# raadyn/aztotmd

Hardware: AMD Instinct MI355X
Metric: ns_per_day (higher is better)
Workload: dtype f64; 1 GPU; 1 000 188 Ar, LJ rc 8.5 A, FCC 63^3 a=5.735 jitter 0.15, dt 1 fs, NVE, init_vel zero (BASELINE config '1 000 000 Ar LJ', SURVEY C4); n_atoms=1000188, n_cells=68921, decomposition=single GPU, transport=single GPU, rccl_ranks=0, pair_variant=0, sort_interval=105, sort_violations=0, pair_lists=1, cells_without_list=0, kernel_timing=off

## Files before the change

### aztotmd_amd/api.py

```python
import ctypes as C
import enum
import os
import subprocess

import numpy as np

_HERE = os.path.dirname(os.path.abspath(__file__))
_LIB = None

STAT_FIELDS = ("step", "time", "engTot", "engKin", "engVdW", "engCoul", "engElecField", "engTemp", "engPot", "temperature",
               "posMom", "negMom", "posCross", "negCross", "pressure", "pairs_dropped", "n_cells", "nose_chit", "nose_conint",
               "engBond", "engAngle", "engCoulRec", "engCoulConst", "sort_interval", "sort_violations", "pair_lists", "cells_without_list", "rebuilds", "skin")


class AztotError(RuntimeError):
    def __init__(self, code, msg):
        super().__init__("aztot error %d: %s" % (code, msg))
        self.code = code


class _Species(C.Structure):
    _fields_ = [("name", C.c_char * 8), ("mass_amu", C.c_double), ("charge", C.c_double), ("frozen", C.c_int32),
                ("radA", C.c_double), ("radB", C.c_double), ("mxEng", C.c_double)]

# ... 85 lines not shown
EXPORTS = ("aztot_device_count", "aztot_device_synchronize", "aztot_init_md", "aztot_model_create", "aztot_model_set_bonded", "aztot_model_query", "aztot_model_species_name", "aztot_model_nucleus_name", "aztot_free_md", "aztot_default_options",
           "aztot_init_device", "aztot_free_device", "aztot_step", "aztot_sync", "aztot_forces", "aztot_get_stats", "aztot_species_crossings", "aztot_md_to_host",
           "aztot_set_state", "aztot_get_clock", "aztot_set_clock", "aztot_cell_table", "aztot_kernel_times", "aztot_reset_kernel_times", "aztot_set_profile", "aztot_comm_id_bytes", "aztot_comm_make_id", "aztot_comm_selftest", "aztot_comm_ranks",
           "aztot_init_device_slab", "aztot_rdf_setup", "aztot_rdf_sample", "aztot_rdf_reset", "aztot_rdf_shape", "aztot_rdf_counts", "aztot_rdf_values",
           "aztot_cn_setup", "aztot_cn_sample", "aztot_cn_shape", "aztot_cn_per_atom", "aztot_cn_table",
           "aztot_tcf_setup", "aztot_tcf_sample", "aztot_tcf_reset", "aztot_tcf_shape", "aztot_tcf_sums", "aztot_tcf_values",
           "aztot_stress_setup", "aztot_stress_sample", "aztot_stress_get", "aztot_stress_per_atom",
           "aztot_adf_setup", "aztot_adf_sample", "aztot_adf_reset", "aztot_adf_shape", "aztot_adf_edges", "aztot_adf_counts", "aztot_adf_values",
           "aztot_adf_neighbours",
           "aztot_sk_setup", "aztot_sk_sample", "aztot_sk_reset", "aztot_sk_shape", "aztot_sk_vectors", "aztot_sk_amplitudes", "aztot_sk_sums", "aztot_sk_values",
           "aztot_boo_setup", "aztot_boo_sample", "aztot_boo_reset", "aztot_boo_shape", "aztot_boo_per_atom", "aztot_boo_qlm", "aztot_boo_counts", "aztot_boo_values",
           "aztot_last_error", "aztot_version")

RDF_KINDS = {"species": 0, "nuclei": 1}
CN_KINDS = {"species": 0, "nuclei": 1}


class DebugBit(enum.IntFlag):
    DBG_BUILD_PHASE_MASK = 3
    DBG_ALWAYS_CLEANUP = 4
    DBG_FOLD_DRIFT = 8
    DBG_NO_FOLD_DRIFT = 16
    DBG_WIDE_ENTRIES = 32
    DBG_KICK_EVERY_STEP = 128
    DBG_LARGE_KICK_PATH = 256
    DBG_GENERIC_PAIR = 512
    DBG_KEEP_VDW_CUT_TEST = 1024
    DBG_STAGE_ONLY = 2048
    DBG_SLAB_GRAPH = 4096
    DBG_FIXED_INTERVAL = 8192
    DBG_OVERLAP_HALO = 16384
    DBG_NO_LISTS = 32768
    DBG_SHORT_LISTS = 65536
    DBG_NO_FUSE_NEXT = 131072
    DBG_FUSE_NEXT = 262144
    DBG_CHECK_EVERY_ATOM = 524288
    DBG_LIST_STATS = 2097152
    DBG_KICK_POST_SPLIT = 4194304
    DBG_GRAPH_ALWAYS = 8388608
    DBG_PLAIN_ONE_ATOM = 16777216
    DBG_NO_BOUNDARY_RADI = 33554432
    DBG_ONE_WAVE_PER_CELL = 67108864
    DBG_ENERGIES_EVERY_STEP = 134217728
    DBG_SETTLE_EVERY_CALL = 268435456
    DBG_NO_FOLD_KICK = 536870912
    DBG_FOLD_KICK = 1073741824
# ... 662 lines not shown
```

### aztotmd_amd/csrc/device_md.h

```cpp
#pragma once
#include <cstdint>

namespace aztot {

constexpr int kSpecCap = 16;

struct AtomArrays
{
    double *x, *y, *z;
    double *vx, *vy, *vz;
    double *fx, *fy, *fz;
    double *U, *rad;
    int32_t *type;
    int32_t *id;
};

struct RefPos { double *x, *y, *z; };

struct SpecTable
{
    double mass[kSpecCap], charge[kSpecCap], rMhdt[kSpecCap];
    double radA[kSpecCap], radB[kSpecCap], mxEng[kSpecCap];
    int32_t charged[kSpecCap], frozen[kSpecCap];
};
// ... 41 lines not shown
    const EwaldG* groups;
    double* T;
    int32_t nK, nW, nG, kx, ky, kz, nBlocksA;
    double* partial;
    double* S;
    double scale, scale2;
};

struct SplitArgs
{
    int n = 1;
    double *fx = nullptr, *fy = nullptr, *fz = nullptr;
    int32_t* arrived = nullptr;
    int capacity = 0;
};

enum DebugBit : unsigned
{
    DBG_BUILD_PHASE_MASK = 3,
    DBG_ALWAYS_CLEANUP = 4,
    DBG_FOLD_DRIFT = 8,
    DBG_NO_FOLD_DRIFT = 16,
    DBG_WIDE_ENTRIES = 32,
    DBG_KICK_EVERY_STEP = 128,
    DBG_LARGE_KICK_PATH = 256,
    DBG_GENERIC_PAIR = 512,
    DBG_KEEP_VDW_CUT_TEST = 1024,
    DBG_STAGE_ONLY = 2048,
    DBG_SLAB_GRAPH = 4096,
    DBG_FIXED_INTERVAL = 8192,
    DBG_OVERLAP_HALO = 16384,
    DBG_NO_LISTS = 32768,
    DBG_SHORT_LISTS = 65536,
    DBG_NO_FUSE_NEXT = 131072,
    DBG_FUSE_NEXT = 262144,
    DBG_CHECK_EVERY_ATOM = 524288,
    DBG_LIST_STATS = 2097152,
    DBG_KICK_POST_SPLIT = 4194304,
    DBG_GRAPH_ALWAYS = 8388608,
    DBG_PLAIN_ONE_ATOM = 16777216,
    DBG_NO_BOUNDARY_RADI = 33554432,
    DBG_ONE_WAVE_PER_CELL = 67108864,
    DBG_ENERGIES_EVERY_STEP = 134217728,
    DBG_SETTLE_EVERY_CALL = 268435456,
    DBG_NO_FOLD_KICK = 536870912,
    DBG_FOLD_KICK = 1073741824
// ... 99 lines not shown
```

### aztotmd_amd/csrc/engine.hip

```cpp
#include "engine.h"

#include <algorithm>
#include <cmath>
#include <array>
#include <cstring>
#include <cstddef>
#include <cstdio>
#include <cstdlib>
#include <stdexcept>
#include <tuple>

#include "exchange.h"
#include "bonded.hip.h"
#include "ewald.hip.h"
#include "kernels.hip.h"
#include "pair_tile.hip.h"
#include "pair_list.hip.h"
#include "rdf.hip.h"
#include "cn.hip.h"
#include "adf.hip.h"
#include "sk.hip.h"
#include "tcf.hip.h"
#include "slab.hip.h"

// ... 466 lines not shown
    waves = forcedWaves_ ? forcedWaves_ : waves_wanted(density * vol, 0);
    int cand = (int)(density * vol * 1.5) + 64;
    int iters = (int)(partners * 1.25 / list_slices(list_atoms_per_wave(std::min(kWave * waves, (int)(1.6 * perCell) + 6), waves))) + 4;
    cand = std::max(kListMinCand * waves, (cand + 63) & ~63);
    iters = std::max(2 * kListMinIter, (iters + 7) & ~7);
    if (const char* e = std::getenv("AZTOT_CAND_CAP")) cand = std::atoi(e);
    if (const char* e = std::getenv("AZTOT_ITER_CAP")) iters = std::atoi(e);
    try { allocate(cand, iters); }
    catch (const std::exception&)
    {
        (void)hipGetLastError();
        release();
    }
}

void ListStore::allocate(int candCapNew, int iterCapNew)
{
    release();
    const StepParams& P = *P_;
    candCapNew = std::max(kListMinCand * waves, std::min((candCapNew + 63) & ~63, kListCandMax));
    iterCapNew = std::max(kListMinIter, std::min((iterCapNew + 7) & ~7, kListIterMax));
    PairLists probe;
    probe.candCap = probe.candLds = probe.stageLds = candCapNew; probe.iterCap = probe.iterLds = iterCapNew; probe.recBytes = pair_list_rec_bytes(P); probe.waves = waves;
    while (candCapNew > kListMinCand && (pair_list_lds_bytes(P, probe) > ldsMax_ || build_lists_lds_bytes(probe) > ldsMax_))
    {
        candCapNew -= 64;
        probe.candCap = probe.candLds = probe.stageLds = candCapNew;
    }
    while (iterCapNew > 2 * kListMinIter && build_lists_lds_bytes(probe) > ldsMax_) { iterCapNew -= 8; probe.iterCap = probe.iterLds = iterCapNew; }
    const size_t nc = (size_t)P.nCellLocal;
    cand = mem_.alloc<uint32_t>(nc * candCapNew, true, stream_);
    meta = mem_.alloc<int32_t>(4 * nc, false, stream_);
    pairs = mem_.alloc<uint16_t>(nc * (size_t)waves * (size_t)iterCapNew * kWave, true, stream_);
    report = mem_.alloc<int32_t>(LR_COUNT, true, stream_); rel = mem_.alloc<float4>((size_t)capacity_ + kWave, true, stream_);
    candCap = candCapNew; iterCap = iterCapNew;
    candLds = stageLds = candCapNew; iterLds = iterCapNew;
    entryBytes = entryNext = 2;
    {
        std::vector<int32_t> mx(4 * nc, 0);
        const int ncy = P.nc[1], ncz = P.nc[2];
        for (size_t c = 0; c < nc; c++)
        {
            const int cz = (int)(c % ncz), cy = (int)((c / ncz) % ncy), lx = (int)(c / ((size_t)ncy * ncz));
            mx[4 * c] = -1; mx[4 * c + 1] = lx | (cy << 10) | (cz << 20);
        }
        HIP_CHECK(hipMemcpyAsync(meta, mx.data(), sizeof(int32_t) * 4 * nc, hipMemcpyHostToDevice, stream_));
        HIP_CHECK(hipStreamSynchronize(stream_));
    }
    on = true;
    if (std::getenv("AZTOT_VERBOSE"))
        std::fprintf(stderr, "aztot: pair lists for %zu cells: %d candidates, %d iterations per cell (%.1f MB), LDS %zu B (list kernel) / %zu B (builder)\n", nc, candCap, iterCap,
                     (double)(nc * ((size_t)candCap * 4 + (size_t)iterCap * 128)) / 1e6, pair_list_lds_bytes(P, pair_lists()), build_lists_lds_bytes(pair_lists()));
}

void ListStore::regrow(int candCapNew, int iterCapNew)
{
    try { allocate(candCapNew, iterCapNew); }
    catch (const std::exception& e)
    {
        (void)hipGetLastError();
        release();
        if (std::getenv("AZTOT_VERBOSE")) std::fprintf(stderr, "aztot: rank %d: no room for larger pair lists (%s): the run goes on without lists\n", rank_, e.what());
    }
}

void ListStore::release() noexcept
{
    if (stream_) (void)hipStreamSynchronize(stream_);
    mem_.release();
    cand = nullptr; meta = nullptr; pairs = nullptr; report = nullptr; rel = nullptr;
    on = false;
}

PairLists ListStore::pair_lists() const
{
    PairLists pl;
    if (on)
    {
        pl.cand = cand; pl.meta = meta; pl.pairs = pairs; pl.noList = report;
        pl.candCap = candCap; pl.iterCap = iterCap; pl.candLds = candLds; pl.stageLds = stageLds; pl.iterLds = iterLds; pl.recBytes = pair_list_rec_bytes(*P_); pl.waves = waves;
        pl.entryBytes = entryBytes; pl.entryScale = entryBytes == 1 ? 1 : pair_list_entry_scale(*P_);
        pl.rel = rel;
    }
    return pl;
}

int ListStore::tile_records_for(int maxT) const
{
    constexpr size_t kLdsBlock = 1280;
    PairLists L = pair_lists();
    const bool roomy = P_->nranks == 1 && capacity_ <= 2 * kFuseKickMaxAtoms;
    int need = std::max(4 * kWave, std::min(candCap, roomy ? maxT + maxT / 16 + 4 : maxT + maxT / 100 + 1));
    if (maxT <= 255 && P_->nranks == 1 && waves == 1) need = 4 * kWave;
    if (need <= 4 * kWave) return need;
    L.candLds = need;
    const size_t blocks = (pair_list_lds_bytes(*P_, L) + kLdsBlock - 1) / kLdsBlock;
    int best = need;
    for (int c = need + 1; c <= candCap; c++)
    {
        L.candLds = c;
        if ((pair_list_lds_bytes(*P_, L) + kLdsBlock - 1) / kLdsBlock > blocks) break;
        best = c;
    }
    return best;
}

int ListStore::stage_records_for(int maxStaged) const
{
    return std::max(4 * kWave, std::min(candCap, (maxStaged + maxStaged / 16 + 4 + 127) & ~127));
}

void ListStore::lds_for(const int32_t* rep, int& candLdsNew, int& stageLdsNew, int& iterLdsNew) const
{
    candLdsNew = tile_records_for(rep[LR_MAX_TILE]);
    stageLdsNew = stage_records_for(rep[LR_MAX_STAGED]);
    iterLdsNew = std::max(2 * kListMinIter, std::min(iterCap, (rep[LR_MAX_ITERS] + rep[LR_MAX_ITERS] / 8 + 2 + 7) & ~7));
    if (entryNext == 1 && ((iterLdsNew + 15) & ~15) <= iterCap) iterLdsNew = (iterLdsNew + 15) & ~15;
}

bool ListStore::narrow_fits(int maxTile, int candLdsNew, int wavesNew) const
{
    return P_->nranks == 1 && !(P_->debugMask & DBG_WIDE_ENTRIES) && !wideForGood_ && wavesNew == 1 && list_preload(candLdsNew) == 4 && maxTile <= 255;
}

bool ListStore::tighten(const int32_t* rep, bool* formatChanged)
{
    if (formatChanged) *formatChanged = false;
    if (rep[LR_TILE_FULL] != 0 || rep[LR_LIST_FULL] != 0 || rep[LR_KEPT_FULL] != 0 || rep[LR_MAX_STAGED] <= 0) return false;
    int c, s, i;
    lds_for(rep, c, s, i);
    bool changed = false;
    if (entryNext == 2 && narrow_fits(rep[LR_MAX_TILE], std::min(candLds, c), waves))
    {
        entryNext = 1;
        lds_for(rep, c, s, i);
        changed = true;
        if (formatChanged) *formatChanged = true;
    }
    if (c >= candLds && s >= stageLds && i >= iterLds) return changed;
    candLds = std::min(candLds, c); stageLds = std::min(stageLds, s); iterLds = std::min(iterLds, i);
    return true;
}

ListStore::Verdict ListStore::adapt(const int32_t* rep, unsigned debug)
{
    Verdict v;
    const bool frozen = debug & DBG_SHORT_LISTS;
    if (debug & DBG_LIST_STATS)
    {
        std::fprintf(stderr, "aztot: per cell: %.2f list iterations, %.1f candidates staged, %.1f kept, %.2f atoms; %.1f %% of the cells walk more than 16 iterations (%d-byte entries)\n",
                     (double)rep[LR_SUM_ITERS] / rep[LR_RECORDED], (double)rep[LR_SUM_STAGED] / rep[LR_RECORDED], (double)rep[LR_SUM_CANDS] / rep[LR_RECORDED],
                     (double)rep[LR_SUM_ATOMS] / rep[LR_RECORDED], 100.0 * (double)rep[LR_OVER_16] / rep[LR_RECORDED], entryBytes);
        HIP_CHECK(hipMemset(&report[LR_SUM_ITERS], 0, sizeof(int32_t) * 4));
        HIP_CHECK(hipMemset(&report[LR_OVER_16], 0, sizeof(int32_t)));
    }
    HIP_CHECK(hipMemsetAsync(&report[LR_UNLISTED], 0, sizeof(int32_t) * 2, stream_));
    HIP_CHECK(hipMemsetAsync(&report[LR_TILE_FULL], 0, sizeof(int32_t) * 3, stream_));
    const int tileFull = rep[LR_TILE_FULL], keptFull = rep[LR_KEPT_FULL], listFull = rep[LR_LIST_FULL], recorded = rep[LR_RECORDED], unlisted = rep[LR_UNLISTED];
    if (std::getenv("AZTOT_VERBOSE"))
        std::fprintf(stderr, "aztot: lists recorded since the last look: %d cells, %d of them without a list (%d: staging full, %d: tile full, %d: list full); most staged %d of %d (LDS %d), largest tile %d (LDS %d), longest list %d of %d (LDS %d)\n",
                     recorded, unlisted, tileFull, keptFull, listFull, rep[LR_MAX_STAGED], candCap, stageLds, rep[LR_MAX_TILE], candLds, rep[LR_MAX_ITERS], iterCap, iterLds);
    int candLdsNew, stageLdsNew, iterLdsNew;
    lds_for(rep, candLdsNew, stageLdsNew, iterLdsNew);
    if (tileFull > 0) stageLdsNew = std::min(candCap, std::max(stageLdsNew, stageLds + 128));
    if (keptFull > 0) candLdsNew = std::min(candCap, std::max(candLdsNew, candLds + 32));
    if (listFull > 0) iterLdsNew = std::min(iterCap, std::max(iterLdsNew, iterLds + 8));
    if (frozen) { candLdsNew = candLds; stageLdsNew = stageLds; iterLdsNew = iterLds; }
    const int wWant = std::max(waves, waves_wanted((double)rep[LR_MAX_TILE], rep[LR_MAX_ITERS]));
    const int wavesNew = (wWant > waves && !forcedWaves_ && !frozen) ? wWant : waves;
    if (entryNext == 1 && (rep[LR_MAX_TILE] > 255 || keptFull > 0 || !narrow_fits(rep[LR_MAX_TILE], candLdsNew, wavesNew)))
    {
        entryNext = 2; wideForGood_ = true;
        v.rebuild = v.launchChanged = true;
    }
    else if (entryNext == 2 && !frozen && tileFull + keptFull + listFull == 0 && narrow_fits(rep[LR_MAX_TILE], candLdsNew, wavesNew))
    {
        entryNext = 1;
        v.launchChanged = true;
        lds_for(rep, candLdsNew, stageLdsNew, iterLdsNew);
    }
    if (wWant > waves && !forcedWaves_ && !frozen)
    {
        const int itersNew = std::max(2 * kListMinIter, ((int)(rep[LR_MAX_ITERS] * (double)waves / wWant * 1.3) + 8 + 7) & ~7);
        const int candNew = std::max(candCap, kListMinCand * wWant);
        waves = wWant;
        regrow(candNew, itersNew);
        v.rebuild = v.launchChanged = true;
        return v;
    }
    const bool capFull = (tileFull > 0 && stageLds == candCap) || (keptFull > 0 && candLds == candCap) || (listFull > 0 && iterLds == iterCap);
    if (capFull && !frozen && (double)(tileFull + keptFull + listFull) > ((P_->nranks == 1 && growths < 3) ? 0.0 : 0.0005 * (double)recorded))
    {
        const int candNew = tileFull + keptFull > 0 ? std::min(kListCandMax, (candCap * 3 / 2 + 63) & ~63) : candCap;
        const int itersNew = listFull > 0 ? std::min(kListIterMax, (iterCap * 2 + 7) & ~7) : iterCap;
        v.launchChanged = true;
        if (growths < 3 && (candNew > candCap || itersNew > iterCap)) { growths++; regrow(candNew, itersNew); v.rebuild = true; }
    }
    else if (candLdsNew != candLds || stageLdsNew != stageLds || iterLdsNew != iterLds)
    {
        candLds = candLdsNew; stageLds = stageLdsNew; iterLds = iterLdsNew;
        v.launchChanged = true;
    }
    if (on && (double)unlisted > 0.02 * (double)recorded && !frozen && tileFull + keptFull + listFull < unlisted / 2)
    {
        on = false;
        v.launchChanged = true;
    }
    return v;
}

void Engine::upload_bonded()
{
    const Model& m = model_;
    const size_t nb = m.bondA.size(), na = m.angC.size();
    hasBonded_ = (nb + na) > 0;
    if (!hasBonded_) return;
    const int N = m.nAt;
    auto up = [&](const void* src, size_t bytes) {
        void* p = dev_alloc<char>(bytes);
        if (bytes) HIP_CHECK(hipMemcpy(p, src, bytes, hipMemcpyHostToDevice));
        return p;
    };
    std::vector<int32_t> bs(N + 1, 0), as(N + 1, 0);
    for (size_t k = 0; k < nb; k++) { bs[m.bondA[k] + 1]++; bs[m.bondB[k] + 1]++; }
    for (size_t k = 0; k < na; k++) { as[m.angC[k] + 1]++; as[m.angL1[k] + 1]++; as[m.angL2[k] + 1]++; }
    for (int i = 0; i < N; i++) { bs[i + 1] += bs[i]; as[i + 1] += as[i]; }
// ... 1118 lines not shown
```

### aztotmd_amd/csrc/list_store.h

```cpp
#pragma once
#include "device_resources.h"
#include "model.h"

namespace aztot {

struct StepParams; struct PairLists;

struct ListStore
{
    struct Verdict
    {
        bool rebuild = false;
        bool launchChanged = false;
    };

    bool on = false;
    uint32_t* cand = nullptr;
    int32_t* meta = nullptr;
    uint16_t* pairs = nullptr;
    int32_t* report = nullptr;
    float4* rel = nullptr;
    int candCap = 0, iterCap = 0;
    int candLds = 0, iterLds = 0;
    int stageLds = 0;
    int waves = 1;
    int growths = 0;
    int entryBytes = 2, entryNext = 2;

    void create(const StepParams& P, const Model& m, const aztot_options& opt, int capacity, double listRadius, hipStream_t stream, int rank);
    void regrow(int candCap, int iterCap);
    void release() noexcept;
    PairLists pair_lists() const;
    void lds_for(const int32_t* rep, int& candLds, int& stageLds, int& iterLds) const;
    bool tighten(const int32_t* rep, bool* formatChanged = nullptr);
    bool narrow_fits(int maxTile, int candLdsNew, int wavesNew) const;
    void begin_recording() { entryBytes = entryNext; }
    Verdict adapt(const int32_t* rep, unsigned debug);

private:
    void allocate(int candCap, int iterCap);
    int tile_records_for(int maxT) const;
    int stage_records_for(int maxStaged) const;
    int waves_wanted(double tileRecords, int iters) const;
    DeviceArena mem_;
    const StepParams* P_ = nullptr;
    hipStream_t stream_ = nullptr;
    int capacity_ = 0, rank_ = 0;
    int forcedWaves_ = 0;
    bool wideForGood_ = false;
    size_t ldsMax_ = 0;
};

}
```

### aztotmd_amd/csrc/pair_list.hip.h

```cpp
#pragma once
#include <type_traits>
#include "pair_tile.hip.h"

namespace aztot {

constexpr int kListPreload = 5;
constexpr int kListMinCand = 64 * kListPreload;
__host__ __device__ inline int list_preload(int candLds) { return candLds <= 4 * kWave ? 4 : kListPreload; }
constexpr int kListMinIter = 16;
constexpr int kListMaxSlices = 32;

constexpr int kListMaxWaves = 4;
__host__ __device__ inline int list_atoms_per_wave(int nAtoms, int W) { return (nAtoms + W - 1) >> (W >> 1); }
__host__ __device__ inline int list_slices(int nAtomsOfWave) { const int n = kWave / (nAtomsOfWave > 0 ? nAtomsOfWave : 1); return n > kListMaxSlices ? kListMaxSlices : (n < 1 ? 1 : n); }

inline bool pair_list_tab_mode(const StepParams& P) { return P.potSet == POTSET_ONE_FAMILY && !P.single_lj; }
inline size_t pair_list_lds_bytes(const StepParams& P, const PairLists& L)
{
    const bool tab = pair_list_tab_mode(P);
    const bool generic = !P.single_lj && P.potSet == POTSET_GENERIC;
    const bool radii = !P.single_lj && !tab;
    size_t b = (size_t)(L.candLds + 1) * 24;
    if (tab) b += sizeof(double) * kLjSpecMax * kLjSpecMax * kPairTabStride + (((size_t)L.candLds + 1 + 15) & ~(size_t)15);
    if (radii) b += sizeof(double) * (size_t)(L.candLds + 1);
// ... 349 lines not shown
            partials[(size_t)PS_EVDW * maxBlocks + pb] = eV;
            partials[(size_t)PS_ECOUL * maxBlocks + pb] = eC;
        }
        if (dropped != 0.0) partials[(size_t)PS_DROPPED * maxBlocks + pb] += dropped;
    }
    if (ENG && P.fuseKick == KICK_SECOND)
    {
        eK = wave_sum(eK);
        if (lane == 0) partials[(size_t)PS_EKIN * maxBlocks + pb] = 0.5 * eK;
    }
    if (N.xn)
    {
        next_step_finish(P, N, nacc, partials, maxBlocks, pb);
        if (blockIdx.x == 0 && threadIdx.x == 0) { N.st->step += 1; N.st->pendingKick = 0; }
    }
    else if (N.pendingAfter >= 0 && blockIdx.x == 0 && threadIdx.x == 0) N.st->pendingKick = N.pendingAfter;
    if (P.fuseKick == KICK_DRIFT && threadIdx.x == 0)
    {
        if (blockIdx.x == 0) N.st->step += 1;
        for (int b = blockIdx.x; b < N.driftBlocks; b += gridDim.x) partials[(size_t)PS_EFIELD * maxBlocks + b] = 0.0;
    }
}

constexpr int kBuildEntRegs = 8;
struct BuildLds
{
    int capS;
    int nWords;
    int hitCap;
    int nTab;
    __host__ __device__ BuildLds(int stageLds, int iterLds, int waves)
        : capS((stageLds + 127) & ~127), nWords((stageLds + 127) / 128), hitCap(iterLds * kWave * waves), nTab(kWave * waves) {}
    __host__ __device__ bool ent_in_regs() const { return capS <= kBuildEntRegs * kWave; }
    __host__ __device__ size_t ent_hit_bytes() const
    {
        const size_t a = sizeof(uint32_t) * (size_t)capS, b = sizeof(uint16_t) * (size_t)hitCap;
        return ((ent_in_regs() ? (a > b ? a : b) : a + b) + 15) & ~(size_t)15;
    }
    __host__ __device__ size_t bytes() const { return sizeof(float) * 4 * (size_t)capS + ent_hit_bytes() + sizeof(uint32_t) * (size_t)nWords * kWave + sizeof(int32_t) * 3 * (size_t)nTab; }
};

__global__ __launch_bounds__(kWave) void k_build_lists(StepParams P, const int32_t* __restrict__ cellStart, int firstCell, int nCellsRun, PairLists L)
{
    extern __shared__ float ldsBuild[];
    const int W = L.waves;
    const BuildLds G(L.stageLds, L.iterLds, W);
    float4* const tile = (float4*)ldsBuild;
    uint16_t* const remap = (uint16_t*)ldsBuild;
    uint32_t* const tent = (uint32_t*)(tile + G.capS);
    const bool entInRegs = G.ent_in_regs();
    uint16_t* const hits = (uint16_t*)(entInRegs ? tent : tent + G.capS);
    uint32_t* const maskBuf = (uint32_t*)((char*)tent + G.ent_hit_bytes());
    int32_t* const entJ = (int32_t*)(maskBuf + (size_t)G.nWords * kWave);
    int32_t* const entN = entJ + G.nTab;
    int32_t* const entC = entN + G.nTab;

    const int lane = threadIdx.x;
    const int per = (nCellsRun + 7) >> 3;
    const int cr = (blockIdx.x & 7) * per + (blockIdx.x >> 3);
    if (blockIdx.x == 0 && lane == 0) atomicAdd(&L.noList[LR_RECORDED], nCellsRun);
    if (cr >= nCellsRun) return;
    const int cell = firstCell + cr;
    const int ncy = P.nc[1], ncz = P.nc[2];
    const int cxyz = L.meta[4 * cell + 1];
    const int lx = cxyz & 1023, cy = (cxyz >> 10) & 1023, cz = (cxyz >> 20) & 1023;
    const int ib = cellStart[cell], ie = cellStart[cell + 1];
    const int nthis = ie - ib;
    if (nthis == 0) { if (lane == 0) L.meta[4 * cell] = 0; return; }
    auto no_list = [&](int why) { if (lane == 0) { L.meta[4 * cell] = -1; atomicAdd(&L.noList[LR_UNLISTED], 1); atomicAdd(&L.noList[LR_UNLISTED_NOW], 1); if (why != LR_NONE) atomicAdd(&L.noList[why], 1); } };
    if (nthis > kWave * W) { no_list(LR_NONE); return; }
    const int RECB = L.entryScale;
    const int stageLds = L.stageLds;
    const float cs0 = (float)P.csz[0], cs1 = (float)P.csz[1], cs2 = (float)P.csz[2];
    const float pruneF = (float)(P.pruneR2 * (1.0 + 1e-5));
    float bc0, bc1, bc2, bh0, bh1, bh2;
    {
        float lo0 = 3e38f, lo1 = 3e38f, lo2 = 3e38f, hi0 = -3e38f, hi1 = -3e38f, hi2 = -3e38f;
        for (int a = lane; a < nthis; a += kWave)
        {
            const float4 m = L.rel[ib + a];
            lo0 = fminf(lo0, m.x); hi0 = fmaxf(hi0, m.x); lo1 = fminf(lo1, m.y); hi1 = fmaxf(hi1, m.y); lo2 = fminf(lo2, m.z); hi2 = fmaxf(hi2, m.z);
        }
#pragma unroll
        for (int o = kWave >> 1; o >= 1; o >>= 1)
        {
            lo0 = fminf(lo0, __shfl_xor(lo0, o, kWave)); hi0 = fmaxf(hi0, __shfl_xor(hi0, o, kWave));
            lo1 = fminf(lo1, __shfl_xor(lo1, o, kWave)); hi1 = fmaxf(hi1, __shfl_xor(hi1, o, kWave));
            lo2 = fminf(lo2, __shfl_xor(lo2, o, kWave)); hi2 = fmaxf(hi2, __shfl_xor(hi2, o, kWave));
        }
        bc0 = 0.5f * (lo0 + hi0); bh0 = 0.5f * (hi0 - lo0) * 1.000001f + 1e-5f;
        bc1 = 0.5f * (lo1 + hi1); bh1 = 0.5f * (hi1 - lo1) * 1.000001f + 1e-5f;
        bc2 = 0.5f * (lo2 + hi2); bh2 = 0.5f * (hi2 - lo2) * 1.000001f + 1e-5f;
    }
// ... 96 lines not shown
        const uint32_t en = tent[q];
        const int rel = (int)(en & 0x3FFFFFFu) - ib;
        if ((en >> 26) == 0x15u && rel >= 0 && rel < nthis) entJ[rel] = q;
    }
    uint32_t te[kBuildEntRegs];
#pragma unroll
    for (int u = 0; u < kBuildEntRegs; u++) te[u] = (entInRegs && u * kWave < T) ? tent[u * kWave + lane] : 0u;
    __builtin_amdgcn_wave_barrier();
    uint32_t keepAcc = 0u;

    const double h0 = 0.5 * P.csz[0], h1 = 0.5 * P.csz[1], h2 = 0.5 * P.csz[2];
    const double rList = sqrt(P.pruneR2);
    const double ext2 = (h0 + rList) * (h0 + rList) + (h1 + rList) * (h1 + rList) + (h2 + rList) * (h2 + rList);
    const float thrList = (float)(P.pruneR2 + 1.9073486328125e-06 * (4.0 * ext2 + P.pruneR2));
    const int aw = list_atoms_per_wave(nthis, W);
    const int NS = list_slices(aw);
    const int rcpNS = 65536 / NS + 1;
    const int nBlk = (T + 15) >> 4;
    const int nW = (nBlk + 7) >> 3;
    const int c16 = lane & 15, kq = lane >> 4;
    const int permc = (c16 >> 2) + ((c16 & 3) << 2);
    const float* const pa = (const float*)tile + 4 * permc + kq;
    int nIter = 0, hitBase = 0, tooLong = 0;
    for (int g0 = 0; g0 < nthis; g0 += 16)
    {
        const int a = g0 + c16;
        const bool validA = a < nthis;
        float4 me = make_float4(1e18f, 1e18f, 1e18f, 0.f);
        if (validA) me = L.rel[ib + a];
        const float fB = (kq == 0) ? 2.0f * me.x : (kq == 1) ? 2.0f * me.y : (kq == 2) ? 2.0f * me.z : 1.0f;
        const float cAtom = thrList - (me.x * me.x + me.y * me.y + me.z * me.z);
        const float4_t cw = {cAtom, cAtom, cAtom, cAtom};
        const int kSelf = validA ? entJ[a] : -1;
        int h = 0;
        for (int wd = 0; wd < nW; wd++)
        {
            float av[8];
#pragma unroll
            for (int q = 0; q < 8; q++) av[q] = pa[(8 * wd + q) * 64];
            uint32_t miss = 0u;
#pragma unroll
            for (int q = 0; q < 8; q++)
            {
                const float4_t d = __builtin_amdgcn_mfma_f32_16x16x4f32(av[q], fB, cw, 0, 0, 0);
                miss = __builtin_amdgcn_alignbit(miss, __float_as_uint(d[0]), 31);
                miss = __builtin_amdgcn_alignbit(miss, __float_as_uint(d[1]), 31);
                miss = __builtin_amdgcn_alignbit(miss, __float_as_uint(d[2]), 31);
                miss = __builtin_amdgcn_alignbit(miss, __float_as_uint(d[3]), 31);
            }
            uint32_t m = ~miss;
            if (kSelf >= 0 && (kSelf & 3) == kq && (kSelf >> 7) == wd) m &= ~(0x80000000u >> ((kSelf & 127) >> 2));
            maskBuf[wd * kWave + lane] = m;
            h += __popc(m);
            uint32_t any = m;
            any |= (uint32_t)__builtin_amdgcn_update_dpp(0, (int)any, 0x128, 0xF, 0xF, false);
            any |= (uint32_t)__builtin_amdgcn_update_dpp(0, (int)any, 0x124, 0xF, 0xF, false);
            any |= (uint32_t)__builtin_amdgcn_update_dpp(0, (int)any, 0x122, 0xF, 0xF, false);
            any |= (uint32_t)__builtin_amdgcn_update_dpp(0, (int)any, 0x121, 0xF, 0xF, false);
            if (c16 == wd) keepAcc |= any;
        }
        int below = 0, total = 0;
#pragma unroll
        for (int q = 0; q < 4; q++)
        {
            const int hq = __shfl(h, c16 | (q << 4), kWave);
            below += (q < kq) ? hq : 0;
            total += hq;
        }
        if (!validA) total = 0;
        int incl = total;
#pragma unroll
        for (int o = 1; o < 16; o <<= 1) { const int up = __shfl_up(incl, o, 16); if (c16 >= o) incl += up; }
        const int myOff = hitBase + incl - total;
        hitBase += __shfl(incl, 15, 16);
        if (validA && kq == 0) { entN[a] = myOff; entC[a] = total; }
        nIter = max(nIter, ((total + NS - 1) * rcpNS) >> 16);
        if (hitBase > G.hitCap) { tooLong = 1; break; }
        if ((P.debugMask & DBG_BUILD_PHASE_MASK) == 2) continue;
        uint16_t* dst = hits + myOff + below;
        for (int wd = 0; wd < nW; wd++)
        {
            uint32_t cur = maskBuf[wd * kWave + lane];
            const int base = 128 * wd + kq;
            while (cur != 0u)
            {
                const int p = __clz(cur);
                cur &= ~(0x80000000u >> p);
                *dst++ = (uint16_t)(base + p * 4);
            }
        }
        __builtin_amdgcn_wave_barrier();
    }
    if ((P.debugMask & DBG_BUILD_PHASE_MASK) >= 2) return;
    nIter = wave_max_int(nIter);
    bool usable = !tooLong && nIter <= ((P.debugMask & DBG_SHORT_LISTS) ? 14 : L.iterCap);
    int kept = 0;
    if (usable)
    {
        __builtin_amdgcn_wave_barrier();
        uint32_t* const myList = L.cand + (size_t)cell * L.candCap;
        auto keep_chunk = [&](int q0, uint32_t entry) {
            const int q = q0 + lane;
            const uint32_t kw = (uint32_t)__shfl((int)keepAcc, ((q & 3) << 4) | (q >> 7), kWave);
            const bool keep = q < T && ((kw << ((q & 127) >> 2)) & 0x80000000u) != 0u;
            const unsigned long long mask = __ballot(keep);
            if (keep)
            {
                const int n = kept + lanes_below(mask);
                remap[q] = (uint16_t)((n + 1) * RECB);
                myList[n] = entry;
            }
// ... 40 lines not shown
                continue;
            }
            for (int c = 0; c * 8 < nIter; c++)
            {
                uint32_t v[8];
#pragma unroll
                for (int u = 0; u < 8; u++)
                {
                    const int e = (c * 8 + u) * NS + slice;
                    v[u] = (e < cnt) ? (uint32_t)remap[src[e]] : 0u;
                }
                out[c * kWave] = make_uint4(v[0] | (v[1] << 16), v[2] | (v[3] << 16), v[4] | (v[5] << 16), v[6] | (v[7] << 16));
            }
        }
    }
    if (lane == 0)
    {
        L.meta[4 * cell] = usable ? (kept | (nIter << 12) | (NS << 20)) : -1;
        L.meta[4 * cell + 2] = ib;
        L.meta[4 * cell + 3] = nthis | (rcpNS << 12);
        if (T > L.noList[LR_MAX_STAGED]) atomicMax(&L.noList[LR_MAX_STAGED], T);
        if (kept > L.noList[LR_MAX_TILE]) atomicMax(&L.noList[LR_MAX_TILE], kept);
        if (usable && nIter > L.noList[LR_MAX_ITERS]) atomicMax(&L.noList[LR_MAX_ITERS], nIter);
        if (P.debugMask & DBG_LIST_STATS)
        {
            atomicAdd(&L.noList[LR_SUM_ITERS], nIter); atomicAdd(&L.noList[LR_SUM_CANDS], kept); atomicAdd(&L.noList[LR_SUM_ATOMS], nthis); atomicAdd(&L.noList[LR_SUM_STAGED], T);
            if (nIter > 16) atomicAdd(&L.noList[LR_OVER_16], 1);
        }
        if (!usable) { atomicAdd(&L.noList[LR_UNLISTED], 1); atomicAdd(&L.noList[LR_UNLISTED_NOW], 1); atomicAdd(&L.noList[keptFull ? LR_KEPT_FULL : LR_LIST_FULL], 1); }
    }
}

inline void launch_build_lists(const PairLaunch& C, PairRange R, PairLists L)
{
    pair_range_default(C.P, R);
    if (R.n == 0) return;
    const BuildLds G(L.stageLds, L.iterLds, L.waves);
    hipLaunchKernelGGL(k_build_lists, dim3(pair_range_grid(R.n)), dim3(kWave), G.bytes(), C.stream, C.P, C.cellStart, R.first, R.n, L);
}
inline size_t build_lists_lds_bytes(const PairLists& L) { return BuildLds(L.stageLds, L.iterLds, L.waves).bytes(); }

template <int MODE, int VDW>
inline void launch_pair_list_as(const PairLaunch& C, PairRange R, PairLists L, NextStep N, bool energies)
{
    const size_t lds = pair_list_lds_bytes(C.P, L);
    const dim3 grid(pair_range_grid(R.n)), block(kWave * L.waves);
    constexpr bool kCanFuseTstat = !pair_mode_reads_radii(MODE);
    const bool four = list_preload(L.candLds) == 4;
    const bool narrow = L.entryBytes == 1;
    if (narrow && (!four || L.waves != 1)) throw std::runtime_error("k_pair_list: one-byte list entries need one wave per cell and a tile of at most 256 records");
#define AZTOT_LAUNCH_LIST_PRE(E, M, T, G, B) hipLaunchKernelGGL((k_pair_list<MODE, VDW, E, M, T, G, B>), grid, block, lds, C.stream, C.P, C.S, C.pots, C.A, C.cellStart, R.first, R.n, C.partials, C.maxBlocks, C.cnt, R.blockBase, L, N)
#define AZTOT_LAUNCH_LIST(E, M, T) do { if (narrow) AZTOT_LAUNCH_LIST_PRE(E, false, T, 4, 1); else if (four) AZTOT_LAUNCH_LIST_PRE(E, M, T, 4, 2); else AZTOT_LAUNCH_LIST_PRE(E, M, T, kListPreload, 2); } while (0)
    if (N.photons)
    {
        if (energies || !kCanFuseTstat) throw std::runtime_error("k_pair_list: the thermostat cannot be fused into this launch");
        if (L.waves == 1) AZTOT_LAUNCH_LIST(false, false, kCanFuseTstat); else AZTOT_LAUNCH_LIST(false, true, kCanFuseTstat);
    }
    else if (L.waves == 1) { if (energies) AZTOT_LAUNCH_LIST(true, false, false); else AZTOT_LAUNCH_LIST(false, false, false); }
    else { if (energies) AZTOT_LAUNCH_LIST(true, true, false); else AZTOT_LAUNCH_LIST(false, true, false); }
#undef AZTOT_LAUNCH_LIST
#undef AZTOT_LAUNCH_LIST_PRE
}

// ... 19 lines not shown
```

### aztotmd_amd/csrc/pair_tile.hip.h

```cpp
#pragma once
#include "kernels.hip.h"

namespace aztot {

constexpr int kTileCap = 320;
constexpr int kTilePad = 16;
constexpr int kTileLds = kTileCap + kTilePad;
static_assert(kTileLds % 32 == 16, "coordinate arrays must be staggered by half the LDS banks");

typedef float float4_t __attribute__((ext_vector_type(4)));

enum PairMode { PM_GENERIC = 0, PM_ONE_LJ = 1, PM_TAB = 2, PM_TAB_EWALD = 3, PM_ONE_SURK = 4, PM_TAB_FENNELL = 5 };
enum PairVdw { VDW_ANY = 0, VDW_LNJS = 1, VDW_BUCK = 2, VDW_P746 = 3, VDW_BMHS = 4, VDW_MIXED = 5, VDW_LJ_NOCUT = 6, VDW_SURK = 7 };
constexpr bool pair_mode_has_table(int mode) { return mode == PM_TAB || mode == PM_TAB_EWALD || mode == PM_TAB_FENNELL; }
constexpr bool pair_mode_reads_radii(int mode) { return mode == PM_GENERIC || mode == PM_ONE_SURK; }
constexpr bool pair_mode_one_species(int mode) { return mode == PM_ONE_LJ || mode == PM_ONE_SURK; }
constexpr bool pair_mode_ewald(int mode) { return mode == PM_TAB_EWALD; }
constexpr bool pair_mode_fennell(int mode) { return mode == PM_TAB_FENNELL; }
constexpr bool pair_vdw_is_lj(int vdw) { return vdw == VDW_LNJS || vdw == VDW_LJ_NOCUT; }
constexpr bool pair_vdw_no_cut_test(int vdw) { return vdw == VDW_LJ_NOCUT; }
constexpr bool pair_vdw_mixed(int vdw) { return vdw == VDW_MIXED; }


inline bool pair_tile_supported(const StepParams& P)
// ... 283 lines not shown
            if (!pair_mode_one_species(MODE)) tj = ttyp[k];
            if (pair_mode_reads_radii(MODE)) radj = trad[k];
            pair_body<MODE, VDW>(P, S, pots, lj, pairTab, live, dx, dy, dz, r2, ti, tj, radi, radj, ljDropR2, nDropHalf, ra, pair_hot(P, lj));
            }
        } while (__any((cur | nxt | lst | ult) != 0u));
    }

    if (MODE != PM_GENERIC) acc.dropped += 0.5 * (double)nDropHalf;
}

enum ListReport : int
{
    LR_UNLISTED = 0,
    LR_RECORDED = 1,
    LR_UNLISTED_NOW = 2,
    LR_MAX_TILE = 3,
    LR_MAX_ITERS = 4,
    LR_TILE_FULL = 5,
    LR_LIST_FULL = 6,
    LR_KEPT_FULL = 7,
    LR_SUM_ITERS = 8, LR_SUM_CANDS = 9, LR_SUM_ATOMS = 10, LR_SUM_STAGED = 11,
    LR_MAX_STAGED = 12,
    LR_OVER_16 = 13,
    LR_COUNT = 16,
    LR_NONE = -1
};
struct PairLists
{
    uint32_t* cand = nullptr;
    int32_t* meta = nullptr;
    uint16_t* pairs = nullptr;
    int32_t* noList = nullptr;
    int32_t candCap = 0;
    int32_t iterCap = 0;
    int32_t candLds = 0;
    int32_t stageLds = 0;
    int32_t iterLds = 0;
    int32_t waves = 1;
    int32_t recBytes = 0;
    int32_t entryScale = 0;
    int32_t entryBytes = 2;
    const float4* rel = nullptr;
};
__device__ __forceinline__ bool list_usable(const PairLists& L, int header) { return header >= 0 && (header & 0xFFF) <= L.candLds; }

__device__ __forceinline__ int wave_max_int(int v)
{
#pragma unroll
    for (int o = kWave >> 1; o >= 1; o >>= 1) v = max(v, __shfl_xor(v, o, kWave));
    return v;
}

struct NextStep
{
    double *xn = nullptr, *yn = nullptr, *zn = nullptr;
    RefPos R0{};
    DevStats* st = nullptr;
    Counts* cnt = nullptr;
    const double *photons = nullptr, *uvx = nullptr, *uvy = nullptr, *uvz = nullptr;
    int pendingAfter = -1;
// ... 466 lines not shown
```

Measured before the change: 904.2 ns/day.

## Split list builder into filter-all-groups then compact phases with per-group mask buffers

The pair-list builder now filters every 16-atom group into its own LDS mask buffer first, then compacts hits in a second pass. The compaction offsets come from per-quarter counts packed into entJ. Hits share LDS with the no-longer-needed tile region instead of sitting beside it, and the entry-register threshold rises from 8 to 12. The aim is to shorten the dependent filter-then-pop chain per group and cut builder LDS footprint. The cost is a mask buffer sized per group, plus a new no-list fallback when a cell holds more atoms than the allocated groups; this is tracked through new report slots that feed the adaptive sizing.

```diff
diff --git a/aztotmd_amd/api.py b/aztotmd_amd/api.py
--- a/aztotmd_amd/api.py
+++ b/aztotmd_amd/api.py
@@ -131,6 +131,7 @@
     DBG_FOLD_DRIFT = 8
     DBG_NO_FOLD_DRIFT = 16
     DBG_WIDE_ENTRIES = 32
+    DBG_HITS_BESIDE_TILE = 64
     DBG_KICK_EVERY_STEP = 128
     DBG_LARGE_KICK_PATH = 256
     DBG_GENERIC_PAIR = 512
diff --git a/aztotmd_amd/csrc/device_md.h b/aztotmd_amd/csrc/device_md.h
--- a/aztotmd_amd/csrc/device_md.h
+++ b/aztotmd_amd/csrc/device_md.h
@@ -87,6 +87,7 @@
     DBG_FOLD_DRIFT = 8,
     DBG_NO_FOLD_DRIFT = 16,
     DBG_WIDE_ENTRIES = 32,
+    DBG_HITS_BESIDE_TILE = 64,
     DBG_KICK_EVERY_STEP = 128,
     DBG_LARGE_KICK_PATH = 256,
     DBG_GENERIC_PAIR = 512,
diff --git a/aztotmd_amd/csrc/engine.hip b/aztotmd_amd/csrc/engine.hip
--- a/aztotmd_amd/csrc/engine.hip
+++ b/aztotmd_amd/csrc/engine.hip
@@ -512,6 +512,7 @@
     iterCapNew = std::max(kListMinIter, std::min((iterCapNew + 7) & ~7, kListIterMax));
     PairLists probe;
     probe.candCap = probe.candLds = probe.stageLds = candCapNew; probe.iterCap = probe.iterLds = iterCapNew; probe.recBytes = pair_list_rec_bytes(P); probe.waves = waves;
+    probe.buildGroups = (P.debugMask & DBG_HITS_BESIDE_TILE) ? 0 : 1;
     while (candCapNew > kListMinCand && (pair_list_lds_bytes(P, probe) > ldsMax_ || build_lists_lds_bytes(probe) > ldsMax_))
     {
         candCapNew -= 64;
@@ -525,6 +526,7 @@
     report = mem_.alloc<int32_t>(LR_COUNT, true, stream_); rel = mem_.alloc<float4>((size_t)capacity_ + kWave, true, stream_);
     candCap = candCapNew; iterCap = iterCapNew;
     candLds = stageLds = candCapNew; iterLds = iterCapNew;
+    buildGroups = groups_that_fit(4 * waves, stageLds, iterLds);
     entryBytes = entryNext = 2;
     {
         std::vector<int32_t> mx(4 * nc, 0);
@@ -569,6 +571,7 @@
     {
         pl.cand = cand; pl.meta = meta; pl.pairs = pairs; pl.noList = report;
         pl.candCap = candCap; pl.iterCap = iterCap; pl.candLds = candLds; pl.stageLds = stageLds; pl.iterLds = iterLds; pl.recBytes = pair_list_rec_bytes(*P_); pl.waves = waves;
+        pl.buildGroups = buildGroups;
         pl.entryBytes = entryBytes; pl.entryScale = entryBytes == 1 ? 1 : pair_list_entry_scale(*P_);
         pl.rel = rel;
     }
@@ -600,12 +603,30 @@
     return std::max(4 * kWave, std::min(candCap, (maxStaged + maxStaged / 16 + 4 + 127) & ~127));
 }
 
-void ListStore::lds_for(const int32_t* rep, int& candLdsNew, int& stageLdsNew, int& iterLdsNew) const
+int ListStore::groups_that_fit(int want, int stageLdsNew, int iterLdsNew) const
+{
+    if (P_->debugMask & DBG_HITS_BESIDE_TILE) return 0;
+    constexpr size_t kLdsBlock = 1280;
+    PairLists L;
+    L.stageLds = stageLdsNew; L.iterLds = iterLdsNew; L.waves = waves;
+    L.buildGroups = std::max(1, std::min(want, 4 * waves));
+    while (L.buildGroups > 1 && build_lists_lds_bytes(L) > ldsMax_) L.buildGroups--;
+    const size_t blocks = (build_lists_lds_bytes(L) + kLdsBlock - 1) / kLdsBlock;
+    while (L.buildGroups < 4 * waves)
+    {
+        L.buildGroups++;
+        if ((build_lists_lds_bytes(L) + kLdsBlock - 1) / kLdsBlock > blocks || build_lists_lds_bytes(L) > ldsMax_) { L.buildGroups--; break; }
+    }
+    return L.buildGroups;
+}
+
+void ListStore::lds_for(const int32_t* rep, int& candLdsNew, int& stageLdsNew, int& iterLdsNew, int& groupsNew) const
 {
     candLdsNew = tile_records_for(rep[LR_MAX_TILE]);
     stageLdsNew = stage_records_for(rep[LR_MAX_STAGED]);
     iterLdsNew = std::max(2 * kListMinIter, std::min(iterCap, (rep[LR_MAX_ITERS] + rep[LR_MAX_ITERS] / 8 + 2 + 7) & ~7));
     if (entryNext == 1 && ((iterLdsNew + 15) & ~15) <= iterCap) iterLdsNew = (iterLdsNew + 15) & ~15;
+    groupsNew = groups_that_fit((rep[LR_MAX_ATOMS] + 15) / 16, stageLdsNew, iterLdsNew);
 }
 
 bool ListStore::narrow_fits(int maxTile, int candLdsNew, int wavesNew) const
@@ -616,19 +637,22 @@
 bool ListStore::tighten(const int32_t* rep, bool* formatChanged)
 {
     if (formatChanged) *formatChanged = false;
-    if (rep[LR_TILE_FULL] != 0 || rep[LR_LIST_FULL] != 0 || rep[LR_KEPT_FULL] != 0 || rep[LR_MAX_STAGED] <= 0) return false;
-    int c, s, i;
-    lds_for(rep, c, s, i);
+    if (rep[LR_TILE_FULL] != 0 || rep[LR_LIST_FULL] != 0 || rep[LR_KEPT_FULL] != 0 || rep[LR_MASK_FULL] != 0 || rep[LR_MAX_STAGED] <= 0) return false;
+    int c, s, i, g;
+    lds_for(rep, c, s, i, g);
     bool changed = false;
     if (entryNext == 2 && narrow_fits(rep[LR_MAX_TILE], std::min(candLds, c), waves))
     {
         entryNext = 1;
-        lds_for(rep, c, s, i);
+        lds_for(rep, c, s, i, g);
         changed = true;
         if (formatChanged) *formatChanged = true;
     }
-    if (c >= candLds && s >= stageLds && i >= iterLds) return changed;
-    candLds = std::min(candLds, c); stageLds = std::min(stageLds, s); iterLds = std::min(iterLds, i);
+    if (c >= candLds && s >= stageLds && i >= iterLds && g >= buildGroups) return changed;
+    candLds = std::min(candLds, c); stageLds = std::min(stageLds, s); iterLds = std::min(iterLds, i); buildGroups = std::min(buildGroups, g);
+    if (std::getenv("AZTOT_VERBOSE"))
+        std::fprintf(stderr, "aztot: list LDS sized from the first recording: tile %d, staging %d, %d iterations, %d mask groups: %zu B (list kernel) / %zu B (builder)\n", candLds, stageLds, iterLds,
+                     buildGroups, pair_list_lds_bytes(*P_, pair_lists()), build_lists_lds_bytes(pair_lists()));
     return true;
 }
 
@@ -646,16 +670,19 @@
     }
     HIP_CHECK(hipMemsetAsync(&report[LR_UNLISTED], 0, sizeof(int32_t) * 2, stream_));
     HIP_CHECK(hipMemsetAsync(&report[LR_TILE_FULL], 0, sizeof(int32_t) * 3, stream_));
-    const int tileFull = rep[LR_TILE_FULL], keptFull = rep[LR_KEPT_FULL], listFull = rep[LR_LIST_FULL], recorded = rep[LR_RECORDED], unlisted = rep[LR_UNLISTED];
+    HIP_CHECK(hipMemsetAsync(&report[LR_MASK_FULL], 0, sizeof(int32_t), stream_));
+    const int tileFull = rep[LR_TILE_FULL], keptFull = rep[LR_KEPT_FULL], listFull = rep[LR_LIST_FULL], maskFull = rep[LR_MASK_FULL], recorded = rep[LR_RECORDED], unlisted = rep[LR_UNLISTED];
     if (std::getenv("AZTOT_VERBOSE"))
-        std::fprintf(stderr, "aztot: lists recorded since the last look: %d cells, %d of them without a list (%d: staging full, %d: tile full, %d: list full); most staged %d of %d (LDS %d), largest tile %d (LDS %d), longest list %d of %d (LDS %d)\n",
-                     recorded, unlisted, tileFull, keptFull, listFull, rep[LR_MAX_STAGED], candCap, stageLds, rep[LR_MAX_TILE], candLds, rep[LR_MAX_ITERS], iterCap, iterLds);
-    int candLdsNew, stageLdsNew, iterLdsNew;
-    lds_for(rep, candLdsNew, stageLdsNew, iterLdsNew);
+        std::fprintf(stderr, "aztot: lists recorded since the last look: %d cells, %d of them without a list (%d: staging full, %d: tile full, %d: list full, %d: mask buffer full); most staged %d of %d (LDS %d), largest tile %d (LDS %d), longest list %d of %d (LDS %d), most atoms %d (LDS %d groups, builder %zu B)\n",
+                     recorded, unlisted, tileFull, keptFull, listFull, maskFull, rep[LR_MAX_STAGED], candCap, stageLds, rep[LR_MAX_TILE], candLds, rep[LR_MAX_ITERS], iterCap, iterLds, rep[LR_MAX_ATOMS], buildGroups,
+                     build_lists_lds_bytes(pair_lists()));
+    int candLdsNew, stageLdsNew, iterLdsNew, groupsNew;
+    lds_for(rep, candLdsNew, stageLdsNew, iterLdsNew, groupsNew);
     if (tileFull > 0) stageLdsNew = std::min(candCap, std::max(stageLdsNew, stageLds + 128));
     if (keptFull > 0) candLdsNew = std::min(candCap, std::max(candLdsNew, candLds + 32));
     if (listFull > 0) iterLdsNew = std::min(iterCap, std::max(iterLdsNew, iterLds + 8));
-    if (frozen) { candLdsNew = candLds; stageLdsNew = stageLds; iterLdsNew = iterLds; }
+    groupsNew = groups_that_fit((rep[LR_MAX_ATOMS] + 15) / 16, stageLdsNew, iterLdsNew);
+    if (frozen) { candLdsNew = candLds; stageLdsNew = stageLds; iterLdsNew = iterLds; groupsNew = buildGroups; }
     const int wWant = std::max(waves, waves_wanted((double)rep[LR_MAX_TILE], rep[LR_MAX_ITERS]));
     const int wavesNew = (wWant > waves && !forcedWaves_ && !frozen) ? wWant : waves;
     if (entryNext == 1 && (rep[LR_MAX_TILE] > 255 || keptFull > 0 || !narrow_fits(rep[LR_MAX_TILE], candLdsNew, wavesNew)))
@@ -663,11 +690,11 @@
         entryNext = 2; wideForGood_ = true;
         v.rebuild = v.launchChanged = true;
     }
-    else if (entryNext == 2 && !frozen && tileFull + keptFull + listFull == 0 && narrow_fits(rep[LR_MAX_TILE], candLdsNew, wavesNew))
+    else if (entryNext == 2 && !frozen && tileFull + keptFull + listFull + maskFull == 0 && narrow_fits(rep[LR_MAX_TILE], candLdsNew, wavesNew))
     {
         entryNext = 1;
         v.launchChanged = true;
-        lds_for(rep, candLdsNew, stageLdsNew, iterLdsNew);
+        lds_for(rep, candLdsNew, stageLdsNew, iterLdsNew, groupsNew);
     }
     if (wWant > waves && !forcedWaves_ && !frozen)
     {
@@ -686,12 +713,12 @@
         v.launchChanged = true;
         if (growths < 3 && (candNew > candCap || itersNew > iterCap)) { growths++; regrow(candNew, itersNew); v.rebuild = true; }
     }
-    else if (candLdsNew != candLds || stageLdsNew != stageLds || iterLdsNew != iterLds)
-    {
-        candLds = candLdsNew; stageLds = stageLdsNew; iterLds = iterLdsNew;
+    else if (candLdsNew != candLds || stageLdsNew != stageLds || iterLdsNew != iterLds || groupsNew != buildGroups)
+    {
+        candLds = candLdsNew; stageLds = stageLdsNew; iterLds = iterLdsNew; buildGroups = groupsNew;
         v.launchChanged = true;
     }
-    if (on && (double)unlisted > 0.02 * (double)recorded && !frozen && tileFull + keptFull + listFull < unlisted / 2)
+    if (on && (double)unlisted > 0.02 * (double)recorded && !frozen && tileFull + keptFull + listFull + maskFull < unlisted / 2)
     {
         on = false;
         v.launchChanged = true;
diff --git a/aztotmd_amd/csrc/list_store.h b/aztotmd_amd/csrc/list_store.h
--- a/aztotmd_amd/csrc/list_store.h
+++ b/aztotmd_amd/csrc/list_store.h
@@ -23,6 +23,7 @@
     int candCap = 0, iterCap = 0;
     int candLds = 0, iterLds = 0;
     int stageLds = 0;
+    int buildGroups = 0;
     int waves = 1;
     int growths = 0;
     int entryBytes = 2, entryNext = 2;
@@ -31,7 +32,7 @@
     void regrow(int candCap, int iterCap);
     void release() noexcept;
     PairLists pair_lists() const;
-    void lds_for(const int32_t* rep, int& candLds, int& stageLds, int& iterLds) const;
+    void lds_for(const int32_t* rep, int& candLds, int& stageLds, int& iterLds, int& buildGroups) const;
     bool tighten(const int32_t* rep, bool* formatChanged = nullptr);
     bool narrow_fits(int maxTile, int candLdsNew, int wavesNew) const;
     void begin_recording() { entryBytes = entryNext; }
@@ -41,6 +42,7 @@
     void allocate(int candCap, int iterCap);
     int tile_records_for(int maxT) const;
     int stage_records_for(int maxStaged) const;
+    int groups_that_fit(int want, int stageLds, int iterLds) const;
     int waves_wanted(double tileRecords, int iters) const;
     DeviceArena mem_;
     const StepParams* P_ = nullptr;
diff --git a/aztotmd_amd/csrc/pair_list.hip.h b/aztotmd_amd/csrc/pair_list.hip.h
--- a/aztotmd_amd/csrc/pair_list.hip.h
+++ b/aztotmd_amd/csrc/pair_list.hip.h
@@ -395,36 +395,53 @@
     }
 }
 
-constexpr int kBuildEntRegs = 8;
+constexpr int kBuildEntRegsBeside = 8;
+constexpr int kBuildEntRegs = 12;
 struct BuildLds
 {
     int capS;
     int nWords;
     int hitCap;
     int nTab;
-    __host__ __device__ BuildLds(int stageLds, int iterLds, int waves)
-        : capS((stageLds + 127) & ~127), nWords((stageLds + 127) / 128), hitCap(iterLds * kWave * waves), nTab(kWave * waves) {}
-    __host__ __device__ bool ent_in_regs() const { return capS <= kBuildEntRegs * kWave; }
-    __host__ __device__ size_t ent_hit_bytes() const
-    {
-        const size_t a = sizeof(uint32_t) * (size_t)capS, b = sizeof(uint16_t) * (size_t)hitCap;
-        return ((ent_in_regs() ? (a > b ? a : b) : a + b) + 15) & ~(size_t)15;
-    }
-    __host__ __device__ size_t bytes() const { return sizeof(float) * 4 * (size_t)capS + ent_hit_bytes() + sizeof(uint32_t) * (size_t)nWords * kWave + sizeof(int32_t) * 3 * (size_t)nTab; }
+    int groups;
+    __host__ __device__ BuildLds(int stageLds, int iterLds, int waves, int buildGroups)
+        : capS((stageLds + 127) & ~127), nWords((stageLds + 127) / 128), hitCap(iterLds * kWave * waves), nTab(kWave * waves), groups(buildGroups) {}
+    __host__ __device__ bool ent_in_regs() const { return capS <= (beside() ? kBuildEntRegsBeside : kBuildEntRegs) * kWave; }
+    __host__ __device__ bool beside() const { return groups == 0; }
+    __host__ __device__ size_t tile_bytes() const { return sizeof(float) * 4 * (size_t)capS; }
+    __host__ __device__ size_t ent_bytes() const { return sizeof(uint32_t) * (size_t)capS; }
+    __host__ __device__ size_t hit_bytes() const { return (sizeof(uint16_t) * (size_t)hitCap + 15) & ~(size_t)15; }
+    __host__ __device__ size_t remap_bytes() const { return sizeof(uint16_t) * (size_t)capS; }
+    __host__ __device__ size_t mask_bytes() const { return sizeof(uint32_t) * (size_t)nWords * kWave * (size_t)(groups > 0 ? groups : 1); }
+    __host__ __device__ size_t ent_off() const { return beside() || tile_bytes() > remap_bytes() + hit_bytes() ? tile_bytes() : remap_bytes() + hit_bytes(); }
+    __host__ __device__ size_t hit_off() const { return !beside() ? remap_bytes() : ent_in_regs() ? ent_off() : ent_off() + ent_bytes(); }
+    __host__ __device__ size_t mask_off() const
+    {
+        if (!beside()) return ent_in_regs() ? ent_off() : ent_off() + ent_bytes();
+        return ent_off() + (ent_in_regs() ? (ent_bytes() > hit_bytes() ? ent_bytes() : hit_bytes()) : ent_bytes() + hit_bytes());
+    }
+    __host__ __device__ size_t tab_off() const
+    {
+        if (!beside() && ent_in_regs()) return ent_off() + (ent_bytes() > mask_bytes() ? ent_bytes() : mask_bytes());
+        return mask_off() + mask_bytes();
+    }
+    __host__ __device__ size_t bytes() const { return tab_off() + sizeof(int32_t) * 3 * (size_t)nTab; }
 };
 
 __global__ __launch_bounds__(kWave) void k_build_lists(StepParams P, const int32_t* __restrict__ cellStart, int firstCell, int nCellsRun, PairLists L)
 {
     extern __shared__ float ldsBuild[];
     const int W = L.waves;
-    const BuildLds G(L.stageLds, L.iterLds, W);
+    const BuildLds G(L.stageLds, L.iterLds, W, L.buildGroups);
+    char* const lds = (char*)ldsBuild;
     float4* const tile = (float4*)ldsBuild;
     uint16_t* const remap = (uint16_t*)ldsBuild;
-    uint32_t* const tent = (uint32_t*)(tile + G.capS);
+    uint32_t* const tent = (uint32_t*)(lds + G.ent_off());
     const bool entInRegs = G.ent_in_regs();
-    uint16_t* const hits = (uint16_t*)(entInRegs ? tent : tent + G.capS);
-    uint32_t* const maskBuf = (uint32_t*)((char*)tent + G.ent_hit_bytes());
-    int32_t* const entJ = (int32_t*)(maskBuf + (size_t)G.nWords * kWave);
+    const bool beside = G.beside();
+    uint16_t* const hits = (uint16_t*)(lds + G.hit_off());
+    uint32_t* const maskBuf = (uint32_t*)(lds + G.mask_off());
+    int32_t* const entJ = (int32_t*)(lds + G.tab_off());
     int32_t* const entN = entJ + G.nTab;
     int32_t* const entC = entN + G.nTab;
 
@@ -441,7 +458,9 @@
     const int nthis = ie - ib;
     if (nthis == 0) { if (lane == 0) L.meta[4 * cell] = 0; return; }
     auto no_list = [&](int why) { if (lane == 0) { L.meta[4 * cell] = -1; atomicAdd(&L.noList[LR_UNLISTED], 1); atomicAdd(&L.noList[LR_UNLISTED_NOW], 1); if (why != LR_NONE) atomicAdd(&L.noList[why], 1); } };
-    if (nthis > kWave * W) { no_list(LR_NONE); return; }
+    auto report_atoms = [&]() { if (lane == 0 && nthis > L.noList[LR_MAX_ATOMS]) atomicMax(&L.noList[LR_MAX_ATOMS], nthis); };
+    if (nthis > kWave * W) { report_atoms(); no_list(LR_NONE); return; }
+    if (!beside && nthis > 16 * G.groups) { report_atoms(); no_list(LR_MASK_FULL); return; }
     const int RECB = L.entryScale;
     const int stageLds = L.stageLds;
     const float cs0 = (float)P.csz[0], cs1 = (float)P.csz[1], cs2 = (float)P.csz[2];
@@ -584,7 +603,7 @@
     const int permc = (c16 >> 2) + ((c16 & 3) << 2);
     const float* const pa = (const float*)tile + 4 * permc + kq;
     int nIter = 0, hitBase = 0, tooLong = 0;
-    for (int g0 = 0; g0 < nthis; g0 += 16)
+    auto filter_group = [&](int g0, uint32_t* mb) -> int
     {
         const int a = g0 + c16;
         const bool validA = a < nthis;
@@ -612,7 +631,7 @@
             }
             uint32_t m = ~miss;
             if (kSelf >= 0 && (kSelf & 3) == kq && (kSelf >> 7) == wd) m &= ~(0x80000000u >> ((kSelf & 127) >> 2));
-            maskBuf[wd * kWave + lane] = m;
+            mb[wd * kWave + lane] = m;
             h += __popc(m);
             uint32_t any = m;
             any |= (uint32_t)__builtin_amdgcn_update_dpp(0, (int)any, 0x128, 0xF, 0xF, false);
@@ -621,13 +640,14 @@
             any |= (uint32_t)__builtin_amdgcn_update_dpp(0, (int)any, 0x121, 0xF, 0xF, false);
             if (c16 == wd) keepAcc |= any;
         }
-        int below = 0, total = 0;
+        int below = 0, total = 0, quarters = 0;
 #pragma unroll
         for (int q = 0; q < 4; q++)
         {
             const int hq = __shfl(h, c16 | (q << 4), kWave);
             below += (q < kq) ? hq : 0;
             total += hq;
+            if (q < 3) quarters |= hq << (10 * q);
         }
         if (!validA) total = 0;
         int incl = total;
@@ -635,20 +655,55 @@
         for (int o = 1; o < 16; o <<= 1) { const int up = __shfl_up(incl, o, 16); if (c16 >= o) incl += up; }
         const int myOff = hitBase + incl - total;
         hitBase += __shfl(incl, 15, 16);
-        if (validA && kq == 0) { entN[a] = myOff; entC[a] = total; }
+        if (validA && kq == 0) { entJ[a] = quarters; entN[a] = myOff; entC[a] = total; }
         nIter = max(nIter, ((total + NS - 1) * rcpNS) >> 16);
-        if (hitBase > G.hitCap) { tooLong = 1; break; }
-        if ((P.debugMask & DBG_BUILD_PHASE_MASK) == 2) continue;
-        uint16_t* dst = hits + myOff + below;
+        if (hitBase > G.hitCap) tooLong = 1;
+        return myOff + below;
+    };
+    auto pop_group = [&](const uint32_t* mb, int at)
+    {
+        uint16_t* dst = hits + at;
         for (int wd = 0; wd < nW; wd++)
         {
-            uint32_t cur = maskBuf[wd * kWave + lane];
+            uint32_t cur = mb[wd * kWave + lane];
             const int base = 128 * wd + kq;
             while (cur != 0u)
             {
                 const int p = __clz(cur);
                 cur &= ~(0x80000000u >> p);
                 *dst++ = (uint16_t)(base + p * 4);
+            }
+        }
+    };
+    const bool compact = (P.debugMask & DBG_BUILD_PHASE_MASK) != 2;
+    if (beside)
+    {
+        for (int g0 = 0; g0 < nthis && !tooLong; g0 += 16)
+        {
+            const int at = filter_group(g0, maskBuf);
+            if (!tooLong && compact) pop_group(maskBuf, at);
+            __builtin_amdgcn_wave_barrier();
+        }
+    }
+    else
+    {
+        const int groupWords = G.nWords * kWave;
+        uint32_t* mb = maskBuf;
+        for (int g0 = 0; g0 < nthis && !tooLong; g0 += 16, mb += groupWords) filter_group(g0, mb);
+        __builtin_amdgcn_wave_barrier();
+        if (!tooLong && compact)
+        {
+            mb = maskBuf;
+            for (int g0 = 0; g0 < nthis; g0 += 16, mb += groupWords)
+            {
+                const int a = g0 + c16;
+                int at = 0;
+                if (a < nthis)
+                {
+                    const int quarters = entJ[a];
+                    at = entN[a] + (kq > 0 ? quarters & 1023 : 0) + (kq > 1 ? (quarters >> 10) & 1023 : 0) + (kq > 2 ? quarters >> 20 : 0);
+                }
+                pop_group(mb, at);
             }
         }
         __builtin_amdgcn_wave_barrier();
@@ -735,6 +790,7 @@
         if (T > L.noList[LR_MAX_STAGED]) atomicMax(&L.noList[LR_MAX_STAGED], T);
         if (kept > L.noList[LR_MAX_TILE]) atomicMax(&L.noList[LR_MAX_TILE], kept);
         if (usable && nIter > L.noList[LR_MAX_ITERS]) atomicMax(&L.noList[LR_MAX_ITERS], nIter);
+        if (nthis > L.noList[LR_MAX_ATOMS]) atomicMax(&L.noList[LR_MAX_ATOMS], nthis);
         if (P.debugMask & DBG_LIST_STATS)
         {
             atomicAdd(&L.noList[LR_SUM_ITERS], nIter); atomicAdd(&L.noList[LR_SUM_CANDS], kept); atomicAdd(&L.noList[LR_SUM_ATOMS], nthis); atomicAdd(&L.noList[LR_SUM_STAGED], T);
@@ -748,10 +804,10 @@
 {
     pair_range_default(C.P, R);
     if (R.n == 0) return;
-    const BuildLds G(L.stageLds, L.iterLds, L.waves);
+    const BuildLds G(L.stageLds, L.iterLds, L.waves, L.buildGroups);
     hipLaunchKernelGGL(k_build_lists, dim3(pair_range_grid(R.n)), dim3(kWave), G.bytes(), C.stream, C.P, C.cellStart, R.first, R.n, L);
 }
-inline size_t build_lists_lds_bytes(const PairLists& L) { return BuildLds(L.stageLds, L.iterLds, L.waves).bytes(); }
+inline size_t build_lists_lds_bytes(const PairLists& L) { return BuildLds(L.stageLds, L.iterLds, L.waves, L.buildGroups).bytes(); }
 
 template <int MODE, int VDW>
 inline void launch_pair_list_as(const PairLaunch& C, PairRange R, PairLists L, NextStep N, bool energies)
diff --git a/aztotmd_amd/csrc/pair_tile.hip.h b/aztotmd_amd/csrc/pair_tile.hip.h
--- a/aztotmd_amd/csrc/pair_tile.hip.h
+++ b/aztotmd_amd/csrc/pair_tile.hip.h
@@ -329,6 +329,8 @@
     LR_SUM_ITERS = 8, LR_SUM_CANDS = 9, LR_SUM_ATOMS = 10, LR_SUM_STAGED = 11,
     LR_MAX_STAGED = 12,
     LR_OVER_16 = 13,
+    LR_MAX_ATOMS = 14,
+    LR_MASK_FULL = 15,
     LR_COUNT = 16,
     LR_NONE = -1
 };
@@ -343,6 +345,7 @@
     int32_t candLds = 0;
     int32_t stageLds = 0;
     int32_t iterLds = 0;
+    int32_t buildGroups = 0;
     int32_t waves = 1;
     int32_t recBytes = 0;
     int32_t entryScale = 0;
```

New measurement: 915.7 ns/day (median of 6 runs). +1.3%, better.
